# bgmanuel99/Super-Resolution-Images-for-3D-Printing-Defect-Detection

Measured on AMD Instinct MI355X. Metric: 4x-SR MPix/s on 512x512 LR batch, higher is better.
Workload: dtype bf16

## Files before the change

### super-resolution-images-for-3d-printing-defect-detection_amd/csrc/api.hip

```cpp
#include <math.h>
#include <stdio.h>
#include <stdlib.h>
#include <string.h>

#include <memory>

#include "common.h"

void* sr_ctx::dalloc(size_t bytes) {
    void* p = nullptr;
    if (bytes == 0) bytes = 16;
    if (alloc_cap > 0 && cur_bytes + (int64_t)bytes > alloc_cap) {
        err = "allocation of " + std::to_string(bytes) + " bytes exceeds the debug cap (sr_debug_set_alloc_cap)";
        return nullptr;
    }
    hipError_t e = hipMalloc(&p, bytes);
    if (e != hipSuccess) {
        err = std::string("hipMalloc(") + std::to_string(bytes) + "): " + hipGetErrorString(e);
        return nullptr;
    }
    allocs[p] = bytes;
    cur_bytes += (int64_t)bytes;
    if (cur_bytes > peak_bytes) peak_bytes = cur_bytes;
    return p;
// ... 46 lines not shown
    if (ni < 0) { prof_names.push_back(name); ni = (int)prof_names.size() - 1; }
    hipEvent_t e[2];
    for (int k = 0; k < 2; ++k) {
        if (!ev_pool.empty()) { e[k] = ev_pool.back(); ev_pool.pop_back(); }
        else if (hipEventCreate(&e[k]) != hipSuccess) return -1;
    }
    (void)hipEventRecord(e[0], st);
    prof_recs.push_back(ProfRec{ni, e[0], e[1], flops, bytes});
    return (int)prof_recs.size() - 1;
}
void sr_ctx::prof_close(int rec, hipStream_t st) {
    if (rec >= 0) (void)hipEventRecord(prof_recs[rec].e1, st);
}

namespace {

struct Param {
    std::string name; int which; std::vector<int64_t> shape; std::vector<float> host; bool set = false;
    int64_t count() const { int64_t n = 1; for (auto s : shape) n *= s; return n; }
};
struct Ref { int buf = -1; int coff = 0; };
enum OpKind { OP_CONVERT, OP_CONV, OP_ATTN, OP_POOL, OP_GAP, OP_DENSE, OP_TOBLK, OP_SUBSAMPLE, OP_PREPROC };
struct Op {
    OpKind kind = OP_CONV;
    Ref in, out, skip1, skip2;
    int conv = -1;
    int act = SR_ACT_LINEAR; float alpha = 1.f, beta1 = 0.f, beta2 = 0.f; int clip = 0, d2s = 1;
    int dw = -1, db = -1, In = 0, Out = 0;
    int chain = -1, chain_pos = 0;
    int rgbtail = -1;
    int pack_alt = -1;
    int pw2 = -1;
    int proj = -1;
};
struct BufSpec { int C = 0; int mul = 1; int shift = 0; bool vec = false; int Cbuf = 0; int blk = 0; int cshift = 0; int cells = 0; int cat = 0; };
struct ConvPart { std::string name; int cout; float scale = 1.f; };
struct ConvSpec { std::vector<ConvPart> parts; int KS = 3, Cin = 0, Cout = 0; ConvWeights w; int rows_head = 0; };
struct ChainSpec { int conv_a = -1, conv_b = -1; int tail = 0; ChainWeights w; };
struct RgbTailSpec { int conv_b = -1; RgbTailWeights w; };
struct ProjSpec { int conv = -1; ProjWeights w; };
struct Pw2Spec { int conv = -1; int act = 0; Pw2Weights w; };

}

struct sr_model {
    sr_ctx* ctx = nullptr;
    int kind = 0;
    sr_model_cfg cfg{};
    int T = SR_DTYPE_BF16;
    std::vector<Param> params;
    std::vector<ConvSpec> convs;
    std::vector<ChainSpec> chains;
    std::vector<RgbTailSpec> rgbtails;
    std::vector<ProjSpec> projs;
    std::vector<Pw2Spec> pw2s;
    std::vector<BufSpec> bufs;
    std::vector<void*> bufp;
    std::vector<float*> dense_dev;
    std::vector<Op> ops;
    int in_C = 3, out_C = 3, out_mul = 1, out_shift = 0; bool out_vec = false;
    bool finalized = false;
    std::vector<size_t> bufcap;
    std::vector<CellGrid> grid_now;
    std::vector<int> routes;
    struct Tap { float* dst; int64_t cap; };
    std::unordered_map<int, Tap> taps;
    std::vector<std::string> op_names;

    int find_param(const std::string& n, int which) const {
        for (size_t i = 0; i < params.size(); ++i) if (params[i].which == which && params[i].name == n) return (int)i;
        return -1;
    }
    void free_bufs() { for (auto& p : bufp) { if (p) ctx->dfree(p); p = nullptr; } bufcap.assign(bufcap.size(), 0); grid_now.assign(grid_now.size(), CellGrid{}); }
    TensorView view(const Ref& r) const { return r.buf >= 0 ? TensorView{bufp[r.buf], bufs[r.buf].Cbuf, r.coff, bufs[r.buf].blk} : TensorView{}; }
};

namespace {

struct Builder {
    sr_model* m;
    int esz() const { return dtype_size(m->T); }
    int E() const { return 16 / esz(); }
    int buf(int C, int mul = 1, int shift = 0) {
        BufSpec b; b.C = C; b.mul = mul; b.shift = shift; b.Cbuf = round_up(C, 32);
        m->bufs.push_back(b); return (int)m->bufs.size() - 1;
    }
    int vecbuf(int C) { BufSpec b; b.C = C; b.vec = true; b.Cbuf = C; m->bufs.push_back(b); return (int)m->bufs.size() - 1; }
    void add_layer_params(const std::string& name, std::vector<int64_t> kshape) {
        Param k; k.name = name; k.which = SR_WEIGHT_KERNEL; k.shape = kshape; m->params.push_back(k);
        Param b; b.name = name; b.which = SR_WEIGHT_BIAS; b.shape = {kshape.back()}; m->params.push_back(b);
    }
    int conv_spec(std::vector<ConvPart> parts, int KS, int Cin) {
        ConvSpec c; c.parts = parts; c.KS = KS; c.Cin = Cin; c.Cout = 0;
        for (auto& p : parts) { c.Cout += p.cout; add_layer_params(p.name, {KS, KS, Cin, p.cout}); }
        m->convs.push_back(c); return (int)m->convs.size() - 1;
    }
    Op& conv(const std::string& name, int KS, int Cin, int Cout, Ref in, Ref out, int act = SR_ACT_LINEAR) {
        Op o; o.kind = OP_CONV; o.conv = conv_spec({{name, Cout}}, KS, Cin); o.in = in; o.out = out; o.act = act;
        m->ops.push_back(o); return m->ops.back();
    }
    Op& conv_again(int spec, Ref in, Ref out, int act = SR_ACT_LINEAR) {
        Op o; o.kind = OP_CONV; o.conv = spec; o.in = in; o.out = out; o.act = act;
        m->ops.push_back(o); return m->ops.back();
    }
    void self_attention(const std::string& name, int x, int y, int qkv, int ao) {
        const float kscale = m->T == SR_DTYPE_BF16 ? 1.4426950408889634f : 1.f;
        Op p; p.kind = OP_CONV; p.conv = conv_spec({{name + "_f", 8, kscale}, {name + "_g", 8}, {name + "_h", 32}}, 1, 64);
        p.in = {x, 0}; p.out = {qkv, 0};
        if (m->T == SR_DTYPE_BF16 && !m->ops.empty() && m->ops.back().kind == OP_CONV && m->ops.back().out.buf == x && m->ops.back().out.coff == 0) {
            ProjSpec ps; ps.conv = p.conv;
            m->projs.push_back(ps);
            m->ops.back().proj = (int)m->projs.size() - 1;
        }
        m->ops.push_back(p);
        Op a; a.kind = OP_ATTN; a.in = {qkv, 0}; a.out = {ao, 0}; m->ops.push_back(a);
        Op& v = conv(name + "_v", 1, 32, 64, {ao, 0}, {y, 0});
        v.skip1 = {x, 0}; v.beta1 = 1.f;
    }
};

int build_srcnn(sr_model* m) {
    Builder b{m};
    const int C = m->cfg.channels;
    m->in_C = C; m->out_C = C; m->out_mul = 1;
    const int x0 = b.buf(b.E()), c1 = b.buf(96), c2 = b.buf(32);
    m->bufs[x0].Cbuf = b.E();
    Op cv; cv.kind = OP_CONVERT; cv.out = {x0, 0}; m->ops.push_back(cv);
    b.conv("conv2d", 9, C, 96, {x0, 0}, {c1, 0}, SR_ACT_RELU);
    b.conv("conv2d_1", 1, 96, 32, {c1, 0}, {c2, 0}, SR_ACT_RELU);
    if (m->T == SR_DTYPE_F32 && C == 3) {
        Pw2Spec ps; ps.conv = m->ops.back().conv; ps.act = SR_ACT_RELU;
        m->pw2s.push_back(ps);
        m->ops[m->ops.size() - 2].pw2 = (int)m->pw2s.size() - 1;
    }
    b.conv("conv2d_2", 5, 32, C, {c2, 0}, {-2, 0});
    return SR_OK;
}

int build_edsr(sr_model* m) {
    Builder b{m};
    const sr_model_cfg& c = m->cfg;
    const int C = c.channels, F = c.num_filters, s = c.scale_factor;
    if (s != 2 && s != 3 && s != 4) return m->ctx->fail(SR_ERR_INVALID, "Scale factor " + std::to_string(s) + " not supported. Use 2, 3, or 4.");
    m->in_C = C; m->out_C = C; m->out_mul = s;
    int li = 0;
    auto lname = [&]() { std::string n = li == 0 ? "conv2d" : "conv2d_" + std::to_string(li); ++li; return n; };
    const int x0 = b.buf(b.E());
    m->bufs[x0].Cbuf = b.E();
    const int head = b.buf(F), tmp = b.buf(F), ra = b.buf(F), rb = b.buf(F);
    Op cv; cv.kind = OP_CONVERT; cv.out = {x0, 0}; m->ops.push_back(cv);
// ... 290 lines not shown
bool chain_fits(const sr_model* m, size_t oi, int w, bool pack2) {
    const Op& op = m->ops[oi];
    if (op.chain < 0 || op.chain_pos != 0) return false;
    const ChainSpec& ch = m->chains[op.chain];
    return !(ch.tail && tapped(m, oi)) && (m->ctx->chain_mask & (ch.tail ? SR_FUSE_DENSE_TAIL : SR_FUSE_DENSE_MID)) && chain_supported(ch.w, m->view(op.in), pack2 ? 48 : w);
}
bool conv1_stream_fits(const sr_model* m, const Op& op, int w, bool pack2) {
    return (m->ctx->chain_mask & SR_FUSE_CONV1_STREAM) && op.chain < 0 && op.act == SR_ACT_RELU && op.alpha == 1.f && bare_epilogue(op) && op.out.buf == op.in.buf &&
           op.in.coff == 0 && op.out.coff == 64 && conv1_stream_supported(m->convs[op.conv].w, m->view(op.in), pack2 ? 48 : w);
}
bool rgb_tail_fits(const sr_model* m, const Op& op, size_t oi, int B, int h, int w) {
    const ConvWeights& cw = m->convs[op.conv].w;
    return op.rgbtail >= 0 && (m->ctx->chain_mask & SR_FUSE_RGB_TAIL) && !tapped(m, oi) && cw.rows && cw.NT == 4 && cw.Cout == 64 && bare_epilogue(op) &&
           op.act != SR_ACT_TANH && op.out.buf >= 0 && (int64_t)m->bufcap[op.out.buf] >= rgbtail_partial_bytes(B, h, w);
}
bool pw2_fits(const sr_model* m, const Op& op, size_t oi) {
    const ConvWeights& cw = m->convs[op.conv].w;
    return op.pw2 >= 0 && (m->ctx->chain_mask & SR_FUSE_SRCNN_1X1) && !tapped(m, oi) && cw.thin && !cw.few && cw.dtype == SR_DTYPE_F32 && bare_epilogue(op);
}
bool pool_fits(const sr_model* m, const Op& op, size_t oi, int h, int w) {
    if (oi + 1 >= m->ops.size() || op.out.buf < 0) return false;
    const Op& pl = m->ops[oi + 1];
    const ConvWeights& cw = m->convs[op.conv].w;
    return (m->ctx->chain_mask & SR_FUSE_POOL) && m->T == SR_DTYPE_BF16 && pl.kind == OP_POOL && pl.in.buf == op.out.buf && pl.out.buf >= 0 && cw.rows && cw.NT == 4 &&
           cw.CoutP == cw.Cout && bare_epilogue(op) && op.act != SR_ACT_TANH && !tapped(m, oi) && !m->grid_now[op.in.buf].gx && !m->grid_now[op.out.buf].gx &&
           h >= 2 && w >= 2 && m->bufs[pl.out.buf].Cbuf % 8 == 0 && m->bufs[pl.out.buf].Cbuf >= cw.Cout;
}
bool proj_fits(const sr_model* m, const Op& op) {
    const ConvWeights& cw = m->convs[op.conv].w;
    return op.proj >= 0 && (m->ctx->chain_mask & SR_FUSE_ATTN_PROJ) && cw.rows && cw.NT == 4 && cw.Cout / (op.d2s * op.d2s) == 64 && cw.CoutP == cw.Cout &&
           op.out.buf >= 0 && !m->bufs[op.out.buf].blk && op.skip2.buf < 0 && !op.clip && op.act != SR_ACT_TANH && m->bufs[op.out.buf].Cbuf % 4 == 0;
}

void plan_routes(sr_model* m, const Layout& L, int B, int H, int W) {
    std::vector<int>& rt = m->routes;
    rt.resize(m->ops.size());
    for (size_t oi = 0; oi < m->ops.size(); ++oi) rt[oi] = m->ops[oi].kind;
    for (size_t oi = 0; oi < m->ops.size(); ++oi) {
        const Op& op = m->ops[oi];
        if (rt[oi] != OP_CONV) continue;
        int h, w;
        buf_hw(m->bufs[op.in.buf], H, W, &h, &w);
        if (chain_fits(m, oi, w, L.pack2)) { rt[oi] = RT_CHAIN; rt[oi + 1] = RT_CHAIN_SECOND; }
        else if (conv1_stream_fits(m, op, w, L.pack2)) rt[oi] = RT_CONV1_STREAM;
        else if (rgb_tail_fits(m, op, oi, B, h, w)) { rt[oi] = RT_RGB_TAIL; rt[oi + 1] = RT_IN_EPILOGUE; }
        else if (pw2_fits(m, op, oi)) { rt[oi] = RT_PW2; rt[oi + 1] = RT_IN_EPILOGUE; }
        else if (pool_fits(m, op, oi, h, w) || proj_fits(m, op)) rt[oi + 1] = RT_IN_EPILOGUE;
    }
}

}

extern "C" {

int sr_init(int device_id, sr_ctx** out) {
    if (!out) return SR_ERR_INVALID;
    *out = nullptr;
    int n = 0;
    if (hipGetDeviceCount(&n) != hipSuccess || device_id < 0 || device_id >= n) return SR_ERR_HIP;
    if (hipSetDevice(device_id) != hipSuccess) return SR_ERR_HIP;
    sr_ctx* c = new sr_ctx();
    c->device = device_id;
    if (hipEventCreate(&c->ev0) != hipSuccess || hipEventCreate(&c->ev1) != hipSuccess) { delete c; return SR_ERR_HIP; }
    c->zero_page = c->dalloc(sr_ctx::ZERO_PAGE_BYTES);
    if (!c->zero_page) { sr_destroy(c); return SR_ERR_OOM; }
    if (hipMemset(c->zero_page, 0, sr_ctx::ZERO_PAGE_BYTES) != hipSuccess) { sr_destroy(c); return SR_ERR_HIP; }
    *out = c;
    return SR_OK;
}

void sr_destroy(sr_ctx* ctx) {
    DeviceGuard dg_(ctx);
// ... 125 lines not shown
    if (cfg->compute_dtype != SR_DTYPE_F32 && cfg->compute_dtype != SR_DTYPE_BF16)
        return ctx->fail(SR_ERR_INVALID, "compute_dtype must be SR_DTYPE_F32 or SR_DTYPE_BF16");
    std::unique_ptr<sr_model> m(new sr_model());
    m->ctx = ctx; m->kind = kind; m->cfg = *cfg; m->T = cfg->compute_dtype;
    if (m->cfg.channels <= 0) m->cfg.channels = 3;
    if (m->cfg.channels > 16 / dtype_size(m->T))
        return ctx->fail(SR_ERR_INVALID, "channels must fit one 16-byte slice (<= 4 for f32, <= 8 for bf16)");
    int rc;
    switch (kind) {
        case SR_MODEL_SRCNN: rc = build_srcnn(m.get()); break;
        case SR_MODEL_EDSR: rc = build_edsr(m.get()); break;
        case SR_MODEL_ESRGAN_G: rc = build_esrgan(m.get()); break;
        case SR_MODEL_VGG16: rc = build_vgg16(m.get()); break;
        case SR_MODEL_ESRGAN_D: rc = build_discriminator(m.get()); break;
        case SR_MODEL_VGG19_FEATURES: rc = build_vgg19_features(m.get()); break;
        default: return ctx->fail(SR_ERR_INVALID, "unknown model kind");
    }
    if (rc) return rc;
    m->dense_dev.assign(m->params.size(), nullptr);
    *out = m.release();
    return SR_OK;
}

void sr_model_destroy(sr_model* m) {
    DeviceGuard dg_(m ? m->ctx : nullptr);
    if (!m) return;
    (void)hipDeviceSynchronize();
    m->free_bufs();
    for (auto& c : m->convs) conv_free_weights(m->ctx, &c.w);
    for (auto& ch : m->chains) chain_free_weights(m->ctx, &ch.w);
    for (auto& rt : m->rgbtails) rgbtail_free_weights(m->ctx, &rt.w);
    for (auto& pj : m->projs) proj_free_weights(m->ctx, &pj.w);
    for (auto& pw : m->pw2s) pw2_free_weights(m->ctx, &pw.w);
    for (auto& p : m->dense_dev) if (p) m->ctx->dfree(p);
    delete m;
}

int sr_model_release_workspace(sr_model* m) {
    if (!m) return SR_ERR_INVALID;
    DeviceGuard dg_(m->ctx);
    SR_HIP(m->ctx, hipDeviceSynchronize());
    m->free_bufs();
    return SR_OK;
}

static void op_out_view(const sr_model* m, const Op& op, int* C, int* mul, int* shift, int* cshift = nullptr) {
    *C = 0; *mul = 1; *shift = 0;
    if (cshift) *cshift = 0;
    if (op.out.buf < 0) return;
    const BufSpec& b = m->bufs[op.out.buf];
    if (b.vec) return;
    *mul = b.mul; *shift = b.shift;
    if (cshift) *cshift = b.cshift;
    if (op.kind == OP_CONV) { const ConvSpec& cs = m->convs[op.conv]; *C = cs.Cout / (op.d2s * op.d2s); }
    else if (op.kind == OP_ATTN) *C = 32;
    else if (op.kind == OP_TOBLK) *C = 64;
    else *C = b.C;
}

int sr_model_num_ops(sr_model* m) { return m ? (int)m->ops.size() : SR_ERR_INVALID; }

int sr_model_op_info(sr_model* m, int index, const char** name, int* channels, int* mul, int* shift, int* ceil_halvings) {
    if (!m || index < 0 || index >= (int)m->ops.size()) return SR_ERR_INVALID;
    if (m->op_names.size() != m->ops.size()) {
        m->op_names.clear();
        static const char* kinds[] = {"convert", "conv", "attention", "maxpool", "gap", "dense", "to_blocked", "stride2_pick", "vgg_preprocess"};
// ... 75 lines not shown
        if (rc) return rc;
    }
    for (auto& ch : m->chains) {
        chain_free_weights(ctx, &ch.w);
        const ConvSpec& a = m->convs[ch.conv_a], &bq = m->convs[ch.conv_b];
        std::vector<float> ka, ba, kb, bb;
        gather(a, ka, ba);
        gather(bq, kb, bb);
        int rc = chain_pack_weights(ctx, ka.data(), ba.data(), kb.data(), bb.data(), a.Cin / 32, a.Cout / 16, bq.Cout / 16, &ch.w);
        if (rc) return rc;
    }
    for (auto& rt : m->rgbtails) {
        rgbtail_free_weights(ctx, &rt.w);
        const ConvSpec& c2 = m->convs[rt.conv_b];
        std::vector<float> k, bias;
        gather(c2, k, bias);
        int rc = rgbtail_pack_weights(ctx, k.data(), bias.data(), c2.Cout, &rt.w);
        if (rc) return rc;
    }
    for (auto& pj : m->projs) {
        proj_free_weights(ctx, &pj.w);
        const ConvSpec& c1 = m->convs[pj.conv];
        std::vector<float> k, bias;
        gather(c1, k, bias);
        int rc = proj_pack_weights(ctx, k.data(), bias.data(), c1.Cout, &pj.w);
        if (rc) return rc;
    }
    for (auto& pw : m->pw2s) {
        pw2_free_weights(ctx, &pw.w);
        const ConvSpec& c1 = m->convs[pw.conv];
        std::vector<float> k, bias;
        gather(c1, k, bias);
        int rc = pw2_pack_weights(ctx, k.data(), bias.data(), c1.Cin, c1.Cout, pw.act, &pw.w);
        if (rc) return rc;
    }
    for (auto& op : m->ops) {
        if (op.kind != OP_DENSE) continue;
        for (int pi : {op.dw, op.db}) {
            if (m->dense_dev[pi]) ctx->dfree(m->dense_dev[pi]);
            const Param& p = m->params[pi];
            m->dense_dev[pi] = static_cast<float*>(ctx->dalloc(sizeof(float) * p.count()));
            if (!m->dense_dev[pi]) return SR_ERR_OOM;
            SR_HIP(ctx, hipMemcpy(m->dense_dev[pi], p.host.data(), sizeof(float) * p.count(), hipMemcpyHostToDevice));
        }
    }
    m->finalized = true;
    return SR_OK;
}

int sr_model_output_shape(sr_model* m, int B, int H, int W, int C, int64_t out_shape[4]) {
    if (!m || !out_shape) return SR_ERR_INVALID;
    (void)C;
    if (m->out_vec) { out_shape[0] = B; out_shape[1] = m->out_C; out_shape[2] = 1; out_shape[3] = 1; }
    else { out_shape[0] = B; out_shape[1] = ((int64_t)H * m->out_mul) >> m->out_shift; out_shape[2] = ((int64_t)W * m->out_mul) >> m->out_shift; out_shape[3] = m->out_C; }
    return SR_OK;
}

int sr_forward(sr_model* m, const void* x, int io_dtype, int B, int H, int W, int C, void* y, int64_t y_capacity, void* stream) {
    DeviceGuard dg_(m ? m->ctx : nullptr);
    if (!m) return SR_ERR_INVALID;
    sr_ctx* ctx = m->ctx;
    hipStream_t st = static_cast<hipStream_t>(stream);
    if (!m->finalized) return ctx->fail(SR_ERR_STATE, "sr_model_finalize has not been called");
    if (!x || !y) return ctx->fail(SR_ERR_INVALID, "null tensor");
    if (io_dtype != SR_DTYPE_F32 && io_dtype != SR_DTYPE_BF16) return ctx->fail(SR_ERR_INVALID, "io dtype must be f32 or bf16");
    if (io_dtype == SR_DTYPE_BF16 && m->T == SR_DTYPE_F32) return ctx->fail(SR_ERR_INVALID, "an fp32 model takes fp32 tensors");
// ... 63 lines not shown
                for (const Ref& r : {op.out, op.skip1, op.skip2})
                    if (r.buf != -1 && !((r.buf >= 0 ? m->grid_now[r.buf] : CellGrid{}) == g)) same = false;
                if (!same) return ctx->fail(SR_ERR_STATE, "packed small-image layout: producer and consumer disagree");
                const int cB = g.gx ? 1 : B;
                if (g.gx) { h = g.Hv; w = g.Wv; }
                ConvEpilogue ep;
                ep.act = op.act; ep.alpha = op.alpha; ep.clip01 = op.clip; ep.d2s_r = op.d2s; ep.cell_h = g.ch; ep.cell_w = g.cw;
                if (op.skip1.buf >= 0) { ep.skip1 = m->view(op.skip1); ep.beta1 = op.beta1; }
                if (op.skip2.buf >= 0) { ep.skip2 = m->view(op.skip2); ep.beta2 = op.beta2; }
                if (route == RT_RGB_TAIL) {
                    const RgbTailWeights& rt = m->rgbtails[op.rgbtail].w;
                    ep.f2 = &rt; ep.f2_part = static_cast<float*>(po);
                    rc = conv_launch(ctx, cs.w, xin, cB, h, w, TensorView{}, ep, st);
                    if (!rc) rc = rgbtail_finish_launch(ctx, rt, ep.f2_part, cB, h, w, nx->act, nx->alpha, nx->clip, y, m->out_C, 0, io_dtype == SR_DTYPE_F32, st);
                    break;
                }
                if (route == RT_PW2) ep.pw2 = &m->pw2s[op.pw2].w;
                else if (nx && nx->kind == OP_POOL) { ep.pool_out = m->view(nx->out); ep.pool_grid = m->grid_now[nx->out.buf]; }
                else if (nx) { ep.pj = &m->projs[op.proj].w; ep.pj_out = m->view(nx->out); }
                if (op.out.buf == -2) {
                    ep.out_f32 = io_dtype == SR_DTYPE_F32;
                    rc = conv_launch(ctx, cs.w, xin, B, h, w, y, m->out_C, 0, ep, st);
                } else {
                    rc = conv_launch(ctx, cs.w, xin, cB, h, w, route == RT_PW2 ? m->view(nx->out) : vo, ep, st);
                }
                break;
            }
            case OP_CONVERT:
                rc = convert_pad_launch(ctx, x, io_dtype, (int64_t)B * H * W, C, po, T, vo.cs, 1.f, 0.f, st);
                break;
            case OP_PREPROC:
                rc = vgg_preproc_launch(ctx, x, io_dtype, (int64_t)B * H * W, po, T, vo.cs, st);
                break;
            case OP_ATTN:
                rc = attention_launch(ctx, T, vi.p, vi.cs,  8,  0,  16, B, h * w, po, vo.cs, 0, st);
                break;
            case OP_SUBSAMPLE:
                rc = subsample2_launch(ctx, T, vi.p, B, h, w, m->bufs[op.in.buf].C, vi.cs, po, vo.cs, st);
                break;
            case OP_TOBLK: {
                const CellGrid& g = m->grid_now[op.out.buf];
                rc = g.gx ? cell_pack_launch(ctx, vi.p, vi.cs, vi.coff, B, h, w, 64, po, vo.cs, vo.coff, g, st)
                   : L.pack2 ? pack_pairs_launch(ctx, vi.p, vi.cs, vi.coff, B, h, w, 64, po, vo.cs, vo.coff, st)
                             : nhwc_to_blocked_launch(ctx, vi.p, vi.cs, vi.coff, B, h, w, 64, po, vo.cs, vo.coff, st);
                break;
            }
            case OP_POOL:
                rc = maxpool2_launch(ctx, T, vi.p, B, h, w, m->bufs[op.in.buf].C, vi.cs, po, vo.cs, st, m->grid_now[op.in.buf], m->grid_now[op.out.buf]);
                break;
            case OP_GAP:
                rc = gap_launch(ctx, T, vi.p, B, h * w, m->bufs[op.in.buf].C, vi.cs, static_cast<float*>(po), st);
                break;
            case OP_DENSE: {
                const bool f32 = op.out.buf != -2 || io_dtype == SR_DTYPE_F32;
                float* yf = static_cast<float*>(op.out.buf == -2 ? y : po);
                rc = dense_launch(ctx, static_cast<const float*>(vi.p), m->dense_dev[op.dw], m->dense_dev[op.db], B, op.In, op.Out, op.act, f32 ? yf : nullptr,
                                  f32 ? 0 : io_dtype, f32 ? nullptr : y, st);
                break;
            }
        }
        if (rc) return rc;
        if (tapped(m, oi)) {
            int C_, mu, sh, th, tw;
            op_out_view(m, op, &C_, &mu, &sh);
            buf_hw(m->bufs[op.out.buf], H, W, &th, &tw);
            const sr_model::Tap& tp = m->taps.at((int)oi);
            if (tp.cap < (int64_t)B * th * tw * C_) return ctx->fail(SR_ERR_CAPACITY, "tap buffer too small");
            rc = tap_copy_launch(ctx, vo.p, T, vo.blk, vo.cs, vo.coff, B, th, tw, C_, tp.dst, st, L.pack2 && vo.blk);
            if (rc) return rc;
// ... 107 lines not shown

int sr_eltwise_views(sr_ctx* ctx, int op, const sr_view* a, const sr_view* b, float alpha, float beta, const sr_view* out, int64_t npix, int C, void* stream) {
    DeviceGuard dg_(ctx);
    if (!ctx) return SR_ERR_INVALID;
    if (!a || !a->p || !out || !out->p) return ctx->fail(SR_ERR_INVALID, "null tensor");
    for (const sr_view* v : {a, b, out})
        if (v && v->p && (v->coff < 0 || v->cs - v->coff < C)) return ctx->fail(SR_ERR_INVALID, "a view is narrower than its channel count");
    const float* bp = (b && b->p) ? static_cast<const float*>(b->p) + b->coff : nullptr;
    return eltwise_views_launch(ctx, op, static_cast<const float*>(a->p) + a->coff, a->cs, bp, bp ? b->cs : 0, alpha, beta,
                                static_cast<float*>(const_cast<void*>(out->p)) + out->coff, out->cs, npix, C, static_cast<hipStream_t>(stream));
}

int sr_self_attention(sr_ctx* ctx, const void* x, int dtype, int B, int H, int W, int C, const float* wf, const float* bf, const float* wg,
                      const float* bg, const float* wh, const float* bh, const float* wv, const float* bv, void* y, void* stream) {
    DeviceGuard dg_(ctx);
    if (!ctx) return SR_ERR_INVALID;
    hipStream_t st = static_cast<hipStream_t>(stream);
    if (C != 64) return ctx->fail(SR_ERR_INVALID, "SelfAttention kernel is built for channels=64 (d_qk=8, d_v=32)");
    if (dtype != SR_DTYPE_F32 && dtype != SR_DTYPE_BF16) return ctx->fail(SR_ERR_INVALID, "dtype must be f32 or bf16");
    if (B <= 0 || H <= 0 || W <= 0) return ctx->fail(SR_ERR_INVALID, "bad tensor shape");
    const float kscale = dtype == SR_DTYPE_BF16 ? 1.4426950408889634f : 1.f;
    std::vector<float> wp((size_t)64 * 48), bp(48);
    for (int ci = 0; ci < 64; ++ci) {
        for (int co = 0; co < 8; ++co) { wp[(size_t)ci * 48 + co] = kscale * wf[ci * 8 + co]; wp[(size_t)ci * 48 + 8 + co] = wg[ci * 8 + co]; }
        for (int co = 0; co < 32; ++co) wp[(size_t)ci * 48 + 16 + co] = wh[ci * 32 + co];
    }
    for (int co = 0; co < 8; ++co) { bp[co] = bf ? kscale * bf[co] : 0.f; bp[8 + co] = bg ? bg[co] : 0.f; }
    for (int co = 0; co < 32; ++co) bp[16 + co] = bh ? bh[co] : 0.f;
    ConvWeights cp, cv;
    int rc = conv_pack_weights(ctx, wp.data(), bp.data(), 1, 64, 48, dtype, &cp);
    if (rc) return rc;
    rc = conv_pack_weights(ctx, wv, bv, 1, 32, 64, dtype, &cv);
    if (rc) { conv_free_weights(ctx, &cp); return rc; }
    const int esz = dtype_size(dtype);
    const int64_t npix = (int64_t)B * H * W;
    void* qkv = ctx->dalloc((size_t)npix * 64 * esz + 4096);
    void* ao = ctx->dalloc((size_t)npix * 32 * esz + 4096);
    if (!qkv || !ao) rc = SR_ERR_OOM;
    if (!rc) rc = (hipMemsetAsync(qkv, 0, (size_t)npix * 64 * esz, st) == hipSuccess) ? SR_OK : ctx->fail(SR_ERR_HIP, "memset");
    ConvEpilogue e0;
    if (!rc) rc = conv_launch(ctx, cp, TensorView{x, 64, 0}, B, H, W, qkv, 64, 0, e0, st);
    if (!rc) rc = attention_launch(ctx, dtype, qkv, 64, 8, 0, 16, B, H * W, ao, 32, 0, st);
    ConvEpilogue e1;
    e1.skip1 = {x, 64, 0}; e1.beta1 = 1.f;
    if (!rc) rc = conv_launch(ctx, cv, TensorView{ao, 32, 0}, B, H, W, y, 64, 0, e1, st);
    hipError_t e = hipStreamSynchronize(st);
    ctx->dfree(qkv); ctx->dfree(ao);
    conv_free_weights(ctx, &cp); conv_free_weights(ctx, &cv);
    if (!rc && e != hipSuccess) return ctx->fail(SR_ERR_HIP, std::string("self_attention: ") + hipGetErrorString(e));
    return rc;
}

int sr_bicubic(sr_ctx* ctx, const void* x, int dtype, int B, int H, int W, int C, int outH, int outW, void* y, void* stream) {
    DeviceGuard dg_(ctx);
    if (!ctx) return SR_ERR_INVALID;
    if (!x || !y) return ctx->fail(SR_ERR_INVALID, "null tensor");
    return bicubic_launch(ctx, x, dtype, B, H, W, C, outH, outW, y, dtype, C, static_cast<hipStream_t>(stream));
}

int sr_resize(sr_ctx* ctx, const void* x, int dtype, int B, int H, int W, int C, int outH, int outW, int interpolation, void* y, void* stream) {
    DeviceGuard dg_(ctx);
    if (!ctx) return SR_ERR_INVALID;
    if (!x || !y) return ctx->fail(SR_ERR_INVALID, "null tensor");
    return resize_launch(ctx, x, dtype, B, H, W, C, outH, outW, interpolation, y, static_cast<hipStream_t>(stream));
}

int sr_psnr(sr_ctx* ctx, const void* a, const void* b, int B, int H, int W, int C, float max_val, float* out_B, void* stream) {
    DeviceGuard dg_(ctx);
    if (!ctx) return SR_ERR_INVALID;
    if (!a || !b || !out_B) return ctx->fail(SR_ERR_INVALID, "null tensor");
    return psnr_launch(ctx, static_cast<const float*>(a), static_cast<const float*>(b), B, (int64_t)H * W * C, max_val, out_B,
                       static_cast<hipStream_t>(stream));
}

int sr_ssim(sr_ctx* ctx, const void* a, const void* b, int B, int H, int W, int C, float max_val, float* out_B, void* stream) {
    DeviceGuard dg_(ctx);
    if (!ctx) return SR_ERR_INVALID;
    if (!a || !b || !out_B) return ctx->fail(SR_ERR_INVALID, "null tensor");
    return ssim_launch(ctx, static_cast<const float*>(a), static_cast<const float*>(b), B, H, W, C, max_val, out_B,
                       static_cast<hipStream_t>(stream));
}
// ... 139 lines not shown
```

### super-resolution-images-for-3d-printing-defect-detection_amd/csrc/attention.hip

```cpp
#include "common.h"

#include <cstdlib>

namespace {

constexpr int KV_TILE = 64;

template <typename T> struct AT;
template <> struct AT<float>  { static constexpr int PITCH = KV_TILE * 4 + 4; };

struct AttnParams {
    const char* qkv; int64_t cs; int qoff, koff, voff;
    char* o; int64_t o_cs; int o_coff;
    int N;
    const float* knorm;
};

__device__ __forceinline__ float xhalf(float v) { return __shfl_xor(v, 32); }

__global__ void __launch_bounds__(256, 2) attn_f32_kernel(AttnParams p) {
    constexpr int PITCH = AT<float>::PITCH;
    __shared__ __attribute__((aligned(16))) char vt[32 * PITCH];

    const int tid = threadIdx.x, lane = tid & 63, wave = tid >> 6, r = lane & 31, h = lane >> 5;
    const int b = blockIdx.y;
    const int N = p.N;
    const float* base = reinterpret_cast<const float*>(p.qkv) + (int64_t)b * N * p.cs;
    const int q = blockIdx.x * 128 + wave * 32 + r;
    const int qc = q < N ? q : N - 1;

    float qf[4];
    {
        const float* qp = base + (int64_t)qc * p.cs + p.qoff;
#pragma unroll
        for (int j = 0; j < 4; ++j) qf[j] = qp[2 * j + h];
    }

    f32x16 oacc;
#pragma unroll
    for (int e = 0; e < 16; ++e) oacc[e] = 0.f;
    float m_run = -INFINITY, l_run = 0.f;

    const int skey = tid >> 2, soct = tid & 3;

    for (int k0 = 0; k0 < N; k0 += KV_TILE) {
        __syncthreads();
        {
            const int key = k0 + skey;
// ... 50 lines not shown
        float* op = reinterpret_cast<float*>(p.o) + ((int64_t)b * N + q) * p.o_cs + p.o_coff;
#pragma unroll
        for (int g = 0; g < 4; ++g) {
            const int d0 = 8 * g + 4 * h;
            f32x4 t = {oacc[4 * g] * inv, oacc[4 * g + 1] * inv, oacc[4 * g + 2] * inv, oacc[4 * g + 3] * inv};
            *reinterpret_cast<f32x4*>(op + d0) = t;
        }
    }
}

constexpr int KT2 = 128;
constexpr int PITCH2 = KT2 * 2 + 8;

__global__ void __launch_bounds__(64) attn_knorm_kernel(const bf16_t* qkv, int64_t cs, int koff, int N, int ngroups, float* out) {
    const int g = blockIdx.x % ngroups, b = blockIdx.x / ngroups, lane = threadIdx.x;
    const bf16_t* base = qkv + (int64_t)b * N * cs + koff;
    float m = 0.f;
#pragma unroll
    for (int t = 0; t < 2; ++t) {
        const int key = g * 128 + t * 64 + lane;
        if (key < N) {
            const bf16x8 k = *reinterpret_cast<const bf16x8*>(base + (int64_t)key * cs);
            float n2 = 0.f;
#pragma unroll
            for (int e = 0; e < 8; ++e) n2 += (float)k[e] * (float)k[e];
            m = fmaxf(m, n2);
        }
    }
#pragma unroll
    for (int o = 32; o > 0; o >>= 1) m = fmaxf(m, __shfl_xor(m, o));
    if (lane == 0) out[(int64_t)b * ngroups + g] = sqrtf(m);
}

template <int QB>
__global__ void __launch_bounds__(256, 3) attn_bf16_kernel(AttnParams p) {
    __shared__ __attribute__((aligned(16))) char vt[32 * PITCH2];
    const int tid = threadIdx.x, lane = tid & 63, wave = tid >> 6, r = lane & 31, h = lane >> 5;
    const int N = p.N;
    constexpr int QW = 64 * QB * 2;
    const int nqt = (N + QW - 1) / QW;
    const int b = blockIdx.x / nqt, qt = blockIdx.x - b * nqt;
    const bf16_t* base = reinterpret_cast<const bf16_t*>(p.qkv) + (int64_t)b * N * p.cs;
    const int cs = (int)p.cs;
    int qi[QB];
    bf16x8 qb[QB];
#pragma unroll
    for (int j = 0; j < QB; ++j) {
        qi[j] = qt * QW + wave * (32 * QB) + j * 32 + r;
        const int qc = qi[j] < N ? qi[j] : N - 1;
        bf16x8 z = {};
        qb[j] = z;
        if (h == 0) qb[j] = *reinterpret_cast<const bf16x8*>(base + (int64_t)qc * cs + p.qoff);
    }
    float qn2 = 0.f;
#pragma unroll
    for (int j = 0; j < QB; ++j) {
        float n2 = 0.f;
#pragma unroll
        for (int e = 0; e < 8; ++e) n2 += (float)qb[j][e] * (float)qb[j][e];
        qn2 = fmaxf(qn2, n2);
    }
#pragma unroll
    for (int o = 32; o > 0; o >>= 1) qn2 = fmaxf(qn2, __shfl_xor(qn2, o));
    const float qmaxv = sqrtf(qn2) * 1.0009765625f;
    const int* knorm_bits = reinterpret_cast<const int*>(p.knorm) + (int64_t)b * ((N + KT2 - 1) / KT2);
    f32x16 oacc[QB];
    bf16x8 sel = {};
// ... 163 lines not shown
        __syncthreads();
    };
    auto slow_tiles = [&](const int k0, const int sub0, bf16x8 kf) {
        for (int sub = sub0; sub < KT2 / 32; ++sub) {
            const int kb = k0 + sub * 32;
            if (kb >= N) break;
            if (sub != sub0) { kf = knext; knext = load_k(kb + 32); }
            if (kb + 32 <= N) tile(kf, sub, kb, false_c, kb == 0);
            else tile(kf, sub, kb, true_c, kb == 0);
        }
    };

    for (int k0 = 0; k0 < N; k0 += KT2) {
        stage_v(k0);
        int sub = 0;
        bf16x8 kf = knext;
        const bool full = k0 != 0 && k0 + KT2 <= N;
        if (full) {
            const bool guard = !(knorm_bits[k0 / KT2] <= thresh_bits);
#pragma unroll
            for (; sub < KT2 / 32; ++sub) {
                kf = knext;
                knext = load_k(k0 + sub * 32 + 32);
                if (!tile_fast(kf, sub, guard)) break;
            }
        } else {
            knext = load_k(k0 + 32);
        }
        if (sub < KT2 / 32) {
            slow_tiles(k0, sub, kf);
            thresh_bits = thresh_of_wave();
        }
    }
#pragma unroll
    for (int j = 0; j < QB; ++j) {
        const float l0 = __shfl(lacc[j][0], r & 15), l1 = __shfl(lacc[j][1], r & 15);
        const float inv = 1.f / ((r >> 4) ? l1 : l0);
        if (qi[j] < N) {
            bf16_t* op = reinterpret_cast<bf16_t*>(p.o) + ((int64_t)b * N + qi[j]) * p.o_cs + p.o_coff;
#pragma unroll
            for (int g = 0; g < 4; ++g) {
                bf16x4 t = {(bf16_t)(oacc[j][4 * g] * inv), (bf16_t)(oacc[j][4 * g + 1] * inv), (bf16_t)(oacc[j][4 * g + 2] * inv),
                            (bf16_t)(oacc[j][4 * g + 3] * inv)};
                *reinterpret_cast<bf16x4*>(op + 8 * g + 4 * h) = t;
            }
        }
    }
}

}

int attention_launch(sr_ctx* ctx, int dtype, const void* qkv, int64_t cs, int qoff, int koff, int voff, int B, int N,
                     void* o, int64_t o_cs, int o_coff, hipStream_t st) {
    if (B <= 0 || N <= 0) return ctx->fail(SR_ERR_INVALID, "attention: empty tensor");
    const int esz = dtype_size(dtype);
    if ((cs * esz) % 16 || (qoff * esz) % 16 || (koff * esz) % 16 || (voff * esz) % 16 || (o_cs * esz) % 16 || (o_coff * esz) % 16)
        return ctx->fail(SR_ERR_INVALID, "attention: views must be 16-byte aligned");
    AttnParams p{static_cast<const char*>(qkv), cs, qoff, koff, voff, static_cast<char*>(o), o_cs, o_coff, N, nullptr};
    dim3 grid((unsigned)((N + 127) / 128), (unsigned)B);
    if (dtype != SR_DTYPE_BF16 && dtype != SR_DTYPE_F32) return ctx->fail(SR_ERR_INVALID, "attention: dtype must be f32 or bf16");
    const int rec = ctx->prof_open(dtype == SR_DTYPE_BF16 ? "attn<bf16>" : "attn<f32>", 2.0 * B * (double)N * N * 40.0,
                                   (double)B * N * 80.0 * esz, st);
    if (dtype == SR_DTYPE_BF16) {
        constexpr int QBr = 2;
        const int64_t nwg = (int64_t)B * ((N + 128 * QBr - 1) / (128 * QBr));
        const int ngroups = (N + KT2 - 1) / KT2;
        if (nwg >= (1ll << 31) || (int64_t)B * ngroups >= (1ll << 31)) { ctx->prof_close(rec, st); return ctx->fail(SR_ERR_INVALID, "attention: too many workgroups for one launch"); }
        float* kn = static_cast<float*>(ctx->arena(ctx->attn_kn, sizeof(float) * (size_t)B * ngroups, st));
        if (!kn) { ctx->prof_close(rec, st); return SR_ERR_OOM; }
        p.knorm = kn;
        hipLaunchKernelGGL(attn_knorm_kernel, dim3((unsigned)((int64_t)B * ngroups)), dim3(64), 0, st, reinterpret_cast<const bf16_t*>(qkv) + 0, cs, koff, N, ngroups, kn);
        hipLaunchKernelGGL(attn_bf16_kernel<QBr>, dim3((unsigned)nwg), dim3(256), 0, st, p);
    }
    else hipLaunchKernelGGL(attn_f32_kernel, grid, dim3(256), 0, st, p);
    ctx->prof_close(rec, st);
    SR_HIP(ctx, hipGetLastError());
    return SR_OK;
}
```

### super-resolution-images-for-3d-printing-defect-detection_amd/csrc/common.h

```cpp
#pragma once
#include <hip/hip_runtime.h>
#include <stdint.h>
#include <string>
#include <unordered_map>
#include <unordered_set>
#include <vector>

#include "../../include/sr355.h"

typedef __bf16 bf16_t;
typedef __bf16 bf16x8 __attribute__((ext_vector_type(8)));
typedef __bf16 bf16x4 __attribute__((ext_vector_type(4)));
typedef float f32x4 __attribute__((ext_vector_type(4)));
typedef float f32x16 __attribute__((ext_vector_type(16)));

struct sr_ctx {
    int device = 0;
    std::string err;
    int64_t cur_bytes = 0, peak_bytes = 0;
    std::unordered_map<void*, size_t> allocs;
    hipEvent_t ev0 = nullptr, ev1 = nullptr;
    bool timed = false;

    void* scratch_buf = nullptr;
// ... 144 lines not shown
                      int dtype, ConvWeights* out, int rows_head = 0);
void conv_free_weights(sr_ctx* ctx, ConvWeights* w);
int conv_launch(sr_ctx* ctx, const ConvWeights& w, TensorView x, int B, int H, int W,
                void* y, int64_t y_cs, int y_coff, const ConvEpilogue& ep, hipStream_t st);
int conv_launch(sr_ctx* ctx, const ConvWeights& w, TensorView x, int B, int H, int W, TensorView y, const ConvEpilogue& ep, hipStream_t st);

int proj_pack_weights(sr_ctx* ctx, const float* w_hwio, const float* bias, int cout, ProjWeights* out);
int pw2_pack_weights(sr_ctx* ctx, const float* w_hwio, const float* bias, int cin, int cout, int act, Pw2Weights* out);
void pw2_free_weights(sr_ctx* ctx, Pw2Weights* w);
void proj_free_weights(sr_ctx* ctx, ProjWeights* w);
int rgbtail_pack_weights(sr_ctx* ctx, const float* w2_hwio, const float* bias2, int c2, RgbTailWeights* out);
void rgbtail_free_weights(sr_ctx* ctx, RgbTailWeights* w);
int64_t rgbtail_partial_bytes(int B, int H, int W);
int rgbtail_finish_launch(sr_ctx* ctx, const RgbTailWeights& w, const float* part, int B, int H, int W, int act, float alpha, int clip01, void* y,
                          int64_t y_cs, int y_coff, int out_f32, hipStream_t st);

struct ChainWeights {
    void* w = nullptr; float* bias = nullptr;
    int ext = 0, nb0 = 0, nb1 = 0;
    size_t bytes = 0;
};
int chain_pack_weights(sr_ctx* ctx, const float* wa_hwio, const float* ba, const float* wb_hwio, const float* bb, int ext, int nb0, int nb1, ChainWeights* out);
void chain_free_weights(sr_ctx* ctx, ChainWeights* w);
bool chain_supported(const ChainWeights& w, const TensorView& in, int W);
bool conv1_stream_supported(const ConvWeights& w, const TensorView& in, int W);
int conv1_stream_launch(sr_ctx* ctx, const ConvWeights& w, TensorView in, int B, int H, int W, hipStream_t st, bool seam = false);
int pack_pairs_launch(sr_ctx* ctx, const void* src, int64_t src_cs, int src_coff, int B, int H, int W, int C, void* dst, int64_t dst_C, int dst_coff, hipStream_t st);
int unpack_pairs_launch(sr_ctx* ctx, const void* src, int64_t src_C, int src_coff, int B, int H, int W, int C, void* dst, int64_t dst_C, int dst_coff, hipStream_t st);
int cell_pack_launch(sr_ctx* ctx, const void* src, int64_t src_cs, int src_coff, int B, int H, int W, int C, void* dst, int64_t dst_C, int dst_coff, const CellGrid& g, hipStream_t st);
int cell_unpack_launch(sr_ctx* ctx, const void* src, int64_t src_C, int src_coff, int B, int H, int W, int C, void* dst, int64_t dst_C, int dst_coff, const CellGrid& g, hipStream_t st);
int chain_launch(sr_ctx* ctx, const ChainWeights& w, TensorView in, int B, int H, int W, TensorView out, TensorView skip_o, float alpha, float beta_x,
                 float beta_o, hipStream_t st, bool seam = false);

int attention_launch(sr_ctx* ctx, int dtype, const void* qkv, int64_t cs, int qoff, int koff, int voff,
                     int B, int N, void* o, int64_t o_cs, int o_coff, hipStream_t st);

int nhwc_to_blocked_launch(sr_ctx* ctx, const void* src, int64_t src_cs, int src_coff, int B, int H, int W, int C, void* dst, int64_t dst_C,
                           int dst_coff, hipStream_t st);
int clock_probe_launch(sr_ctx* ctx, float* mhz_out, hipStream_t st);
int tap_copy_launch(sr_ctx* ctx, const void* src, int dtype, int blk, int64_t cs, int coff, int B, int H, int W, int C, float* dst, hipStream_t st, bool pairs = false);
int convert_pad_launch(sr_ctx* ctx, const void* x, int in_dtype, int64_t npix, int C, void* y, int out_dtype,
                       int Cp, float mul, float add, hipStream_t st);
int maxpool2_launch(sr_ctx* ctx, int dtype, const void* x, int B, int H, int W, int C, int64_t x_cs, void* y,
                    int64_t y_cs, hipStream_t st, CellGrid in_grid = CellGrid{}, CellGrid out_grid = CellGrid{});
int gap_launch(sr_ctx* ctx, int dtype, const void* x, int B, int HW, int C, int64_t x_cs, float* y, hipStream_t st);
int dense_launch(sr_ctx* ctx, const float* x, const float* w, const float* bias, int B, int In, int Out, int act,
                 float* y, int y_dtype, void* y_typed, hipStream_t st);
int bicubic_launch(sr_ctx* ctx, const void* x, int dtype, int B, int H, int W, int C, int outH, int outW,
                   void* y, int out_dtype, int64_t y_cs, hipStream_t st);
int subsample2_launch(sr_ctx* ctx, int dtype, const void* x, int B, int H, int W, int C, int64_t x_cs, void* y, int64_t y_cs, hipStream_t st);
int vgg_preproc_launch(sr_ctx* ctx, const void* x, int in_dtype, int64_t npix, void* y, int out_dtype, int Cp, hipStream_t st);
int l1_launch(sr_ctx* ctx, const float* a, const float* b, int64_t n, float* out, hipStream_t st);
int spectral_l1_launch(sr_ctx* ctx, const float* a, const float* b, int B, int H, int W, int C, float* out, hipStream_t st);
int wgrad_launch(sr_ctx* ctx, const float* x, const float* dy, int B, int H, int W, int Cin, int Cout, int KS, float* dw, float* db, hipStream_t st);
int wgrad_launch_views(sr_ctx* ctx, const float* x, int64_t x_cs, const float* dy, int64_t dy_cs, int B, int H, int W, int Cin, int Cout, int KS, float* dw, float* db,
                       hipStream_t st);
int eltwise_views_launch(sr_ctx* ctx, int op, const float* a, int64_t a_cs, const float* b, int64_t b_cs, float alpha, float beta, float* out, int64_t o_cs, int64_t npix, int C,
                         hipStream_t st);
int adam_launch(sr_ctx* ctx, float* w, const float* g, float* m, float* v, int64_t n, float lr_t, float b1, float omb1, float b2, float omb2, float eps,
                float gscale, hipStream_t st);
int eltwise_launch(sr_ctx* ctx, int op, const float* a, const float* b, float alpha, float beta, float* out, int64_t n, hipStream_t st);
int space_to_depth_launch(sr_ctx* ctx, const float* x, int B, int H, int W, int C, int r, float* y, hipStream_t st);
int matmul_launch(sr_ctx* ctx, const float* A, const float* B, float* C, int batch, int M, int N, int K, int tA, int tB, float alpha, hipStream_t st);
int softmax_rows_launch(sr_ctx* ctx, float* s, int64_t rows, int cols, hipStream_t st);
int softmax_bwd_launch(sr_ctx* ctx, const float* p, const float* dp, float* ds, int64_t rows, int cols, hipStream_t st);
int maxpool2_bwd_launch(sr_ctx* ctx, const float* x, const float* dy, int B, int H, int W, int C, float* dx, hipStream_t st);
int zero_insert2_launch(sr_ctx* ctx, const float* dy, int B, int H, int W, int C, float* out, hipStream_t st);
int spectral_l1_bwd_launch(sr_ctx* ctx, const float* a, const float* b, int B, int H, int W, int C, float scale, float* da, hipStream_t st);
// ... 17 lines not shown
```

Before: 111.6.

## Fuse attention output 1x1 projection and residual into bf16 attention kernel

New measurement: 111.9 (median of 6 runs). Within noise of the previous version (+0.3%).

```diff
diff --git a/super-resolution-images-for-3d-printing-defect-detection_amd/csrc/api.hip b/super-resolution-images-for-3d-printing-defect-detection_amd/csrc/api.hip
--- a/super-resolution-images-for-3d-printing-defect-detection_amd/csrc/api.hip
+++ b/super-resolution-images-for-3d-printing-defect-detection_amd/csrc/api.hip
@@ -102,6 +102,7 @@
     int pack_alt = -1;
     int pw2 = -1;
     int proj = -1;
+    int atail = -1;
 };
 struct BufSpec { int C = 0; int mul = 1; int shift = 0; bool vec = false; int Cbuf = 0; int blk = 0; int cshift = 0; int cells = 0; int cat = 0; };
 struct ConvPart { std::string name; int cout; float scale = 1.f; };
@@ -110,6 +111,7 @@
 struct RgbTailSpec { int conv_b = -1; RgbTailWeights w; };
 struct ProjSpec { int conv = -1; ProjWeights w; };
 struct Pw2Spec { int conv = -1; int act = 0; Pw2Weights w; };
+struct AttnTailSpec { int conv = -1; AttnTailWeights w; };
 
 }
 
@@ -124,6 +126,7 @@
     std::vector<RgbTailSpec> rgbtails;
     std::vector<ProjSpec> projs;
     std::vector<Pw2Spec> pw2s;
+    std::vector<AttnTailSpec> atails;
     std::vector<BufSpec> bufs;
     std::vector<void*> bufp;
     std::vector<float*> dense_dev;
@@ -186,6 +189,11 @@
         Op a; a.kind = OP_ATTN; a.in = {qkv, 0}; a.out = {ao, 0}; m->ops.push_back(a);
         Op& v = conv(name + "_v", 1, 32, 64, {ao, 0}, {y, 0});
         v.skip1 = {x, 0}; v.beta1 = 1.f;
+        if (m->T == SR_DTYPE_BF16) {
+            AttnTailSpec ts; ts.conv = v.conv;
+            m->atails.push_back(ts);
+            m->ops[m->ops.size() - 2].atail = (int)m->atails.size() - 1;
+        }
     }
 };
 
@@ -542,12 +550,24 @@
            op.out.buf >= 0 && !m->bufs[op.out.buf].blk && op.skip2.buf < 0 && !op.clip && op.act != SR_ACT_TANH && m->bufs[op.out.buf].Cbuf % 4 == 0;
 }
 
+bool attn_tail_fits(const sr_model* m, size_t oi) {
+    const Op& op = m->ops[oi];
+    if (op.atail < 0 || oi + 1 >= m->ops.size() || m->T != SR_DTYPE_BF16 || !(m->ctx->chain_mask & SR_FUSE_ATTN_PROJ) || tapped(m, oi)) return false;
+    const Op& v = m->ops[oi + 1];
+    if (v.kind != OP_CONV || v.conv != m->atails[op.atail].conv || v.in.buf != op.out.buf || v.in.coff != 0 || v.out.buf < 0 || v.skip1.buf < 0 || v.skip2.buf >= 0) return false;
+    if (v.act != SR_ACT_LINEAR || v.alpha != 1.f || v.beta1 != 1.f || v.clip || v.d2s != 1) return false;
+    for (int bi : {op.in.buf, v.out.buf, v.skip1.buf})
+        if (m->bufs[bi].blk || m->grid_now[bi].gx || m->bufs[bi].Cbuf % 8 != 0) return false;
+    return true;
+}
+
 void plan_routes(sr_model* m, const Layout& L, int B, int H, int W) {
     std::vector<int>& rt = m->routes;
     rt.resize(m->ops.size());
     for (size_t oi = 0; oi < m->ops.size(); ++oi) rt[oi] = m->ops[oi].kind;
     for (size_t oi = 0; oi < m->ops.size(); ++oi) {
         const Op& op = m->ops[oi];
+        if (rt[oi] == OP_ATTN && attn_tail_fits(m, oi)) rt[oi + 1] = RT_IN_EPILOGUE;
         if (rt[oi] != OP_CONV) continue;
         int h, w;
         buf_hw(m->bufs[op.in.buf], H, W, &h, &w);
@@ -739,6 +759,7 @@
     for (auto& rt : m->rgbtails) rgbtail_free_weights(m->ctx, &rt.w);
     for (auto& pj : m->projs) proj_free_weights(m->ctx, &pj.w);
     for (auto& pw : m->pw2s) pw2_free_weights(m->ctx, &pw.w);
+    for (auto& at : m->atails) attn_tail_free_weights(m->ctx, &at.w);
     for (auto& p : m->dense_dev) if (p) m->ctx->dfree(p);
     delete m;
 }
@@ -880,6 +901,14 @@
         std::vector<float> k, bias;
         gather(c1, k, bias);
         int rc = pw2_pack_weights(ctx, k.data(), bias.data(), c1.Cin, c1.Cout, pw.act, &pw.w);
+        if (rc) return rc;
+    }
+    for (auto& at : m->atails) {
+        attn_tail_free_weights(ctx, &at.w);
+        const ConvSpec& cv = m->convs[at.conv];
+        std::vector<float> k, bias;
+        gather(cv, k, bias);
+        int rc = attn_tail_pack_weights(ctx, k.data(), bias.data(), &at.w);
         if (rc) return rc;
     }
     for (auto& op : m->ops) {
@@ -1009,9 +1038,12 @@
             case OP_PREPROC:
                 rc = vgg_preproc_launch(ctx, x, io_dtype, (int64_t)B * H * W, po, T, vo.cs, st);
                 break;
-            case OP_ATTN:
-                rc = attention_launch(ctx, T, vi.p, vi.cs,  8,  0,  16, B, h * w, po, vo.cs, 0, st);
+            case OP_ATTN: {
+                AttnTail tl;
+                if (nx) { tl.w = &m->atails[op.atail].w; tl.x = m->view(nx->skip1); tl.y = m->view(nx->out); }
+                rc = attention_launch(ctx, T, vi.p, vi.cs,  8,  0,  16, B, h * w, po, vo.cs, 0, st, nx ? &tl : nullptr);
                 break;
+            }
             case OP_SUBSAMPLE:
                 rc = subsample2_launch(ctx, T, vi.p, B, h, w, m->bufs[op.in.buf].C, vi.cs, po, vo.cs, st);
                 break;
@@ -1185,6 +1217,9 @@
     if (rc) return rc;
     rc = conv_pack_weights(ctx, wv, bv, 1, 32, 64, dtype, &cv);
     if (rc) { conv_free_weights(ctx, &cp); return rc; }
+    AttnTailWeights tw;
+    const bool fuse_tail = dtype == SR_DTYPE_BF16 && (ctx->chain_mask & SR_FUSE_ATTN_PROJ);
+    if (fuse_tail && (rc = attn_tail_pack_weights(ctx, wv, bv, &tw))) { conv_free_weights(ctx, &cp); conv_free_weights(ctx, &cv); return rc; }
     const int esz = dtype_size(dtype);
     const int64_t npix = (int64_t)B * H * W;
     void* qkv = ctx->dalloc((size_t)npix * 64 * esz + 4096);
@@ -1193,13 +1228,16 @@
     if (!rc) rc = (hipMemsetAsync(qkv, 0, (size_t)npix * 64 * esz, st) == hipSuccess) ? SR_OK : ctx->fail(SR_ERR_HIP, "memset");
     ConvEpilogue e0;
     if (!rc) rc = conv_launch(ctx, cp, TensorView{x, 64, 0}, B, H, W, qkv, 64, 0, e0, st);
-    if (!rc) rc = attention_launch(ctx, dtype, qkv, 64, 8, 0, 16, B, H * W, ao, 32, 0, st);
+    AttnTail tl;
+    tl.w = &tw; tl.x = TensorView{x, 64, 0}; tl.y = TensorView{y, 64, 0};
+    if (!rc) rc = attention_launch(ctx, dtype, qkv, 64, 8, 0, 16, B, H * W, ao, 32, 0, st, fuse_tail ? &tl : nullptr);
     ConvEpilogue e1;
     e1.skip1 = {x, 64, 0}; e1.beta1 = 1.f;
-    if (!rc) rc = conv_launch(ctx, cv, TensorView{ao, 32, 0}, B, H, W, y, 64, 0, e1, st);
+    if (!rc && !fuse_tail) rc = conv_launch(ctx, cv, TensorView{ao, 32, 0}, B, H, W, y, 64, 0, e1, st);
     hipError_t e = hipStreamSynchronize(st);
     ctx->dfree(qkv); ctx->dfree(ao);
     conv_free_weights(ctx, &cp); conv_free_weights(ctx, &cv);
+    attn_tail_free_weights(ctx, &tw);
     if (!rc && e != hipSuccess) return ctx->fail(SR_ERR_HIP, std::string("self_attention: ") + hipGetErrorString(e));
     return rc;
 }
diff --git a/super-resolution-images-for-3d-printing-defect-detection_amd/csrc/attention.hip b/super-resolution-images-for-3d-printing-defect-detection_amd/csrc/attention.hip
--- a/super-resolution-images-for-3d-printing-defect-detection_amd/csrc/attention.hip
+++ b/super-resolution-images-for-3d-printing-defect-detection_amd/csrc/attention.hip
@@ -1,6 +1,7 @@
 #include "common.h"
 
 #include <cstdlib>
+#include <cstring>
 
 namespace {
 
@@ -14,6 +15,9 @@
     char* o; int64_t o_cs; int o_coff;
     int N;
     const float* knorm;
+    const char* wv; const float* bv;
+    const char* x; int64_t x_cs; int x_coff;
+    char* y; int64_t y_cs; int y_coff;
 };
 
 __device__ __forceinline__ float xhalf(float v) { return __shfl_xor(v, 32); }
@@ -130,7 +134,7 @@
     if (lane == 0) out[(int64_t)b * ngroups + g] = sqrtf(m);
 }
 
-template <int QB>
+template <int QB, bool TAIL>
 __global__ void __launch_bounds__(256, 3) attn_bf16_kernel(AttnParams p) {
     __shared__ __attribute__((aligned(16))) char vt[32 * PITCH2];
     const int tid = threadIdx.x, lane = tid & 63, wave = tid >> 6, r = lane & 31, h = lane >> 5;
@@ -360,6 +364,71 @@
             thresh_bits = thresh_of_wave();
         }
     }
+    if constexpr (TAIL) {
+        int lane, r, h;
+        asm volatile("v_mbcnt_lo_u32_b32 %0, -1, 0\n\tv_mbcnt_hi_u32_b32 %0, -1, %0" : "=v"(lane));
+        r = lane & 31; h = lane >> 5;
+        const int q0 = qt * QW + __builtin_amdgcn_readfirstlane(wave) * (32 * QB) + r;
+        bf16x8 wv[2][2];
+#pragma unroll
+        for (int cb = 0; cb < 2; ++cb)
+#pragma unroll
+            for (int ks = 0; ks < 2; ++ks) wv[cb][ks] = *reinterpret_cast<const bf16x8*>(p.wv + ((cb * 2 + ks) * 64 + lane) * 16);
+        bf16x8 xs[QB][2][2];
+        f32x4 bias[2][2][2];
+#pragma unroll
+        for (int cb = 0; cb < 2; ++cb)
+#pragma unroll
+            for (int pr = 0; pr < 2; ++pr) {
+                const int c0 = 32 * cb + 16 * pr + 8 * h;
+#pragma unroll
+                for (int j = 0; j < QB; ++j) {
+                    const int qj = q0 + 32 * j;
+                    const int64_t pix = (int64_t)b * N + (qj < N ? qj : N - 1);
+                    xs[j][cb][pr] = *reinterpret_cast<const bf16x8*>(reinterpret_cast<const bf16_t*>(p.x) + pix * p.x_cs + p.x_coff + c0);
+                }
+                bias[cb][pr][0] = *reinterpret_cast<const f32x4*>(p.bv + c0);
+                bias[cb][pr][1] = *reinterpret_cast<const f32x4*>(p.bv + c0 + 4);
+            }
+#pragma unroll
+        for (int j = 0; j < QB; ++j) {
+            const float l0 = __shfl(lacc[j][0], r & 15), l1 = __shfl(lacc[j][1], r & 15);
+            const float inv = 1.f / ((r >> 4) ? l1 : l0);
+            f32x16 acc[2];
+            {
+                bf16x8 of[2];
+#pragma unroll
+                for (int ks = 0; ks < 2; ++ks)
+#pragma unroll
+                    for (int e = 0; e < 8; ++e) of[ks][e] = (bf16_t)(oacc[j][8 * ks + e] * inv);
+#pragma unroll
+                for (int cb = 0; cb < 2; ++cb) {
+                    acc[cb] = __builtin_amdgcn_mfma_f32_32x32x16_bf16(wv[cb][0], of[0], zero16, 0, 0, 0);
+                    acc[cb] = __builtin_amdgcn_mfma_f32_32x32x16_bf16(wv[cb][1], of[1], acc[cb], 0, 0, 0);
+                }
+            }
+            const int qj = q0 + 32 * j;
+            bf16_t* yp = reinterpret_cast<bf16_t*>(p.y) + ((int64_t)b * N + (qj < N ? qj : N - 1)) * p.y_cs + p.y_coff + 8 * h;
+#pragma unroll
+            for (int cb = 0; cb < 2; ++cb) {
+#pragma unroll
+                for (int pr = 0; pr < 2; ++pr) {
+                    float v[8];
+#pragma unroll
+                    for (int e = 0; e < 4; ++e) {
+                        const float ge = acc[cb][8 * pr + e], go = acc[cb][8 * pr + 4 + e];
+                        const auto sw = __builtin_amdgcn_permlane32_swap(__builtin_bit_cast(unsigned, ge), __builtin_bit_cast(unsigned, go), false, false);
+                        v[e] = __builtin_bit_cast(float, (unsigned)sw[0]);
+                        v[4 + e] = __builtin_bit_cast(float, (unsigned)sw[1]);
+                    }
+                    bf16x8 t;
+#pragma unroll
+                    for (int e = 0; e < 8; ++e) t[e] = (bf16_t)((v[e] + bias[cb][pr][e >> 2][e & 3]) + (float)xs[j][cb][pr][e]);
+                    if (qj < N) *reinterpret_cast<bf16x8*>(yp + 32 * cb + 16 * pr) = t;
+                }
+            }
+        }
+    } else {
 #pragma unroll
     for (int j = 0; j < QB; ++j) {
         const float l0 = __shfl(lacc[j][0], r & 15), l1 = __shfl(lacc[j][1], r & 15);
@@ -374,21 +443,69 @@
             }
         }
     }
-}
-
+    }
+}
+
+uint16_t bf16_bits(float f) {
+    uint32_t u;
+    memcpy(&u, &f, 4);
+    if ((u & 0x7fffffffu) > 0x7f800000u) return (uint16_t)((u >> 16) | 0x40);
+    u += 0x7fffu + ((u >> 16) & 1u);
+    return (uint16_t)(u >> 16);
+}
+
+}
+
+int attn_tail_pack_weights(sr_ctx* ctx, const float* w_hwio, const float* bias, AttnTailWeights* out) {
+    std::vector<uint16_t> host((size_t)4 * 64 * 8);
+    for (int cb = 0; cb < 2; ++cb)
+        for (int ks = 0; ks < 2; ++ks)
+            for (int l = 0; l < 64; ++l)
+                for (int e = 0; e < 8; ++e) {
+                    const int dv = (e & 3) + 8 * (2 * ks + (e >> 2)) + 4 * (l >> 5);
+                    host[((size_t)(cb * 2 + ks) * 64 + l) * 8 + e] = bf16_bits(w_hwio[(size_t)dv * 64 + 32 * cb + (l & 31)]);
+                }
+    AttnTailWeights tw;
+    tw.a = ctx->dalloc(host.size() * 2);
+    if (!tw.a) return SR_ERR_OOM;
+    tw.bias = static_cast<float*>(ctx->dalloc(sizeof(float) * 64));
+    if (!tw.bias) { ctx->dfree(tw.a); return SR_ERR_OOM; }
+    float hb[64];
+    for (int i = 0; i < 64; ++i) hb[i] = bias ? bias[i] : 0.f;
+    SR_HIP(ctx, hipMemcpy(tw.a, host.data(), host.size() * 2, hipMemcpyHostToDevice));
+    SR_HIP(ctx, hipMemcpy(tw.bias, hb, sizeof hb, hipMemcpyHostToDevice));
+    *out = tw;
+    return SR_OK;
+}
+
+void attn_tail_free_weights(sr_ctx* ctx, AttnTailWeights* w) {
+    if (w->a) ctx->dfree(w->a);
+    if (w->bias) ctx->dfree(w->bias);
+    w->a = nullptr; w->bias = nullptr;
 }
 
 int attention_launch(sr_ctx* ctx, int dtype, const void* qkv, int64_t cs, int qoff, int koff, int voff, int B, int N,
-                     void* o, int64_t o_cs, int o_coff, hipStream_t st) {
+                     void* o, int64_t o_cs, int o_coff, hipStream_t st, const AttnTail* tail) {
     if (B <= 0 || N <= 0) return ctx->fail(SR_ERR_INVALID, "attention: empty tensor");
     const int esz = dtype_size(dtype);
     if ((cs * esz) % 16 || (qoff * esz) % 16 || (koff * esz) % 16 || (voff * esz) % 16 || (o_cs * esz) % 16 || (o_coff * esz) % 16)
         return ctx->fail(SR_ERR_INVALID, "attention: views must be 16-byte aligned");
-    AttnParams p{static_cast<const char*>(qkv), cs, qoff, koff, voff, static_cast<char*>(o), o_cs, o_coff, N, nullptr};
+    AttnParams p{static_cast<const char*>(qkv), cs, qoff, koff, voff, static_cast<char*>(o), o_cs, o_coff, N, nullptr, nullptr, nullptr, nullptr, 0, 0, nullptr, 0, 0};
+    if (tail) {
+        if (dtype != SR_DTYPE_BF16) return ctx->fail(SR_ERR_INVALID, "attention: the fused tail is a bf16 path");
+        if (!tail->w || !tail->w->a || !tail->w->bias || !tail->x.p || !tail->y.p || tail->x.blk || tail->y.blk)
+            return ctx->fail(SR_ERR_INVALID, "attention: the fused tail needs packed weights and NHWC views of x and y");
+        if (tail->x.cs % 8 || tail->x.coff % 8 || tail->y.cs % 8 || tail->y.coff % 8 || tail->x.cs - tail->x.coff < 64 || tail->y.cs - tail->y.coff < 64)
+            return ctx->fail(SR_ERR_INVALID, "attention: the fused tail's views must be 16-byte aligned and 64 channels wide");
+        p.wv = static_cast<const char*>(tail->w->a); p.bv = tail->w->bias;
+        p.x = static_cast<const char*>(tail->x.p); p.x_cs = tail->x.cs; p.x_coff = tail->x.coff;
+        p.y = static_cast<char*>(const_cast<void*>(tail->y.p)); p.y_cs = tail->y.cs; p.y_coff = tail->y.coff;
+    }
     dim3 grid((unsigned)((N + 127) / 128), (unsigned)B);
     if (dtype != SR_DTYPE_BF16 && dtype != SR_DTYPE_F32) return ctx->fail(SR_ERR_INVALID, "attention: dtype must be f32 or bf16");
-    const int rec = ctx->prof_open(dtype == SR_DTYPE_BF16 ? "attn<bf16>" : "attn<f32>", 2.0 * B * (double)N * N * 40.0,
-                                   (double)B * N * 80.0 * esz, st);
+    if (ctx->route_log) ctx->route_text += dtype != SR_DTYPE_BF16 ? "attn<f32>\n" : (tail ? "attn<bf16>/tail\n" : "attn<bf16>\n");
+    const int rec = ctx->prof_open(dtype == SR_DTYPE_BF16 ? "attn<bf16>" : "attn<f32>", 2.0 * B * (double)N * N * 40.0 + (tail ? 2.0 * B * (double)N * 32.0 * 64.0 : 0.0),
+                                   (double)B * N * (tail ? 176.0 : 80.0) * esz, st);
     if (dtype == SR_DTYPE_BF16) {
         constexpr int QBr = 2;
         const int64_t nwg = (int64_t)B * ((N + 128 * QBr - 1) / (128 * QBr));
@@ -398,7 +515,8 @@
         if (!kn) { ctx->prof_close(rec, st); return SR_ERR_OOM; }
         p.knorm = kn;
         hipLaunchKernelGGL(attn_knorm_kernel, dim3((unsigned)((int64_t)B * ngroups)), dim3(64), 0, st, reinterpret_cast<const bf16_t*>(qkv) + 0, cs, koff, N, ngroups, kn);
-        hipLaunchKernelGGL(attn_bf16_kernel<QBr>, dim3((unsigned)nwg), dim3(256), 0, st, p);
+        if (tail) hipLaunchKernelGGL((attn_bf16_kernel<QBr, true>), dim3((unsigned)nwg), dim3(256), 0, st, p);
+        else hipLaunchKernelGGL((attn_bf16_kernel<QBr, false>), dim3((unsigned)nwg), dim3(256), 0, st, p);
     }
     else hipLaunchKernelGGL(attn_f32_kernel, grid, dim3(256), 0, st, p);
     ctx->prof_close(rec, st);
diff --git a/super-resolution-images-for-3d-printing-defect-detection_amd/csrc/common.h b/super-resolution-images-for-3d-printing-defect-detection_amd/csrc/common.h
--- a/super-resolution-images-for-3d-printing-defect-detection_amd/csrc/common.h
+++ b/super-resolution-images-for-3d-printing-defect-detection_amd/csrc/common.h
@@ -200,8 +200,15 @@
 int chain_launch(sr_ctx* ctx, const ChainWeights& w, TensorView in, int B, int H, int W, TensorView out, TensorView skip_o, float alpha, float beta_x,
                  float beta_o, hipStream_t st, bool seam = false);
 
+struct AttnTailWeights {
+    void* a = nullptr;
+    float* bias = nullptr;
+};
+struct AttnTail { const AttnTailWeights* w = nullptr; TensorView x, y; };
+int attn_tail_pack_weights(sr_ctx* ctx, const float* w_hwio, const float* bias, AttnTailWeights* out);
+void attn_tail_free_weights(sr_ctx* ctx, AttnTailWeights* w);
 int attention_launch(sr_ctx* ctx, int dtype, const void* qkv, int64_t cs, int qoff, int koff, int voff,
-                     int B, int N, void* o, int64_t o_cs, int o_coff, hipStream_t st);
+                     int B, int N, void* o, int64_t o_cs, int o_coff, hipStream_t st, const AttnTail* tail = nullptr);
 
 int nhwc_to_blocked_launch(sr_ctx* ctx, const void* src, int64_t src_cs, int src_coff, int B, int H, int W, int C, void* dst, int64_t dst_C,
                            int dst_coff, hipStream_t st);
```
